# JeroendenBoef/GraphPOPE

Hardware: AMD Instinct MI355X
Metric: POPE embeddings/sec (nodes x anchors) + SAGE nodes/sec, Flickr 256 anchors (higher is better)
Workload: dtype u64; 1 GPU; configs[1]: flickr-shaped geodesic-stochastic, N=89250 E=899756 F=500, 256 anchors PER GPU (np.random seed 42); inputs resident in HBM (edge_index, x) -> [N, F+K] f32 in HBM on every rank; anchors_total=256, anchors_per_rank=256, parallelism=single GPU

## Files before the change

### graphpope_amd/_lib.py

```python
from __future__ import annotations

import ctypes
import os
from ctypes import c_char_p, c_double, c_float, c_int, c_int32, c_int64, c_size_t, c_uint64, c_void_p, POINTER

_HERE = os.path.dirname(os.path.abspath(__file__))
LIB_PATH = os.path.join(_HERE, "libgraphpope_hip.so")

OK, ERR_INVALID, ERR_HIP, ERR_INDEX, ERR_HOP_OVERFLOW, ERR_WORKSPACE, ERR_NO_DEVICE, ERR_UNSORTED = 0, -1, -2, -3, -4, -5, -6, -7
METRIC = {"distance": 0, "similarity": 1, "euclidean": 2}
KNOB_LIVE_MODE, KNOB_FINALIZE_VARIANT, KNOB_FINALIZE_BLOCKS = 0, 1, 2
KNOB_PAIRWISE_KERNEL, KNOB_COPY_BATCHES, KNOB_FAIL_HOST_REGISTER = 4, 5, 7
KNOB_SAGE_FORWARD_OVERLAP = 14
KNOB_GEMM_TILE16_BUFFERS = 18
KNOB_PREPARE_MERGE = 19
KNOB_STREAMK_XCD = 20
KNOB_FORWARD_WHOLE_TILES = 21

SIGNATURES = {
    "pope_last_error": (c_char_p, []),
    "pope_version": (c_char_p, []),
    "pope_require_device": (c_int, [POINTER(c_int32)]),
    "pope_debug_set": (c_int, [c_int32, c_int32]),
    "pope_host_copy_2d": (c_int, [c_void_p, c_int64, c_void_p, c_int64, c_int64, c_int64, c_int32]),
    "pope_copy_2d_to_host": (c_int, [c_void_p, c_int64, c_void_p, c_int64, c_int64, c_int64, c_void_p]),
    "pope_assemble_host_result": (c_int, [c_void_p, c_int64, c_int64, c_void_p, c_int64, c_int64, c_void_p, c_int64, c_int64, c_int32,
                                          c_int32, c_void_p]),
    "pope_assemble_begin": (c_void_p, [c_void_p, c_int64, c_int64, c_void_p, c_int64, c_int64, c_int32, c_int32]),
    "pope_assemble_finish": (c_int, [c_void_p, c_void_p, c_int64, c_int64, c_void_p]),
    "pope_assemble_abort": (None, [c_void_p]),
    "pope_assemble_prepare": (None, [c_int32]),
    "pope_assemble_ring_ready": (c_int32, []),
    "pope_assemble_finish_codes": (c_int, [c_void_p, c_void_p, c_int64, c_int32, c_void_p, c_void_p]),
    "pope_geodesic_hop_codes": (c_int, [c_void_p, c_int32, c_int32, c_int64, c_int32, c_void_p, c_int64, c_void_p, c_void_p]),
    "pope_host_pin": (c_int, [c_void_p, c_size_t]),
    "pope_host_unpin": (c_int, [c_void_p]),
    "pope_copy_to_device": (c_int, [c_void_p, c_void_p, c_size_t, c_void_p]),
    "pope_csr_scratch_bytes": (c_size_t, [c_int64, c_int64]),
    "pope_csr_aux_elems": (c_size_t, [c_int64]),
    "pope_csr_build": (c_int, [c_void_p, c_int64, c_int64, c_void_p, c_void_p, c_void_p, c_void_p, c_void_p, c_size_t,
# ... 15 lines not shown
    "pope_kmeans_lloyd_step": (c_int, [c_void_p, c_int64, c_int32, c_void_p, c_int32, c_void_p, c_void_p, c_void_p, c_void_p, c_void_p,
                                       c_void_p, c_size_t, c_void_p]),
    "pope_words": (c_int32, [c_int32]),
    "pope_plane_bytes": (c_size_t, [c_int64, c_int32]),
    "pope_bfs_scratch_bytes": (c_size_t, [c_int64, c_int64, c_int32]),
    "pope_geodesic_bfs": (c_int, [c_void_p, c_void_p, c_void_p, c_void_p, c_int64, c_int64, c_void_p, c_int32, c_void_p, c_int32,
                                  c_void_p, c_size_t, POINTER(c_int32), POINTER(c_int32), c_void_p]),
    "pope_geodesic_bfs_begin": (c_int, [c_void_p, c_void_p, c_void_p, c_void_p, c_int64, c_int64, c_void_p, c_int32, c_void_p, c_int32,
                                        c_void_p, c_size_t, c_void_p]),
    "pope_geodesic_bfs_finish": (c_int, [c_void_p, c_void_p, c_void_p, c_void_p, c_int64, c_int64, c_void_p, c_int32, c_void_p, c_int32,
                                         c_void_p, c_size_t, POINTER(c_int32), POINTER(c_int32), c_void_p]),
    "pope_geodesic_finalize": (c_int, [c_void_p, c_int32, c_int64, c_int32, c_void_p, c_int32, c_void_p, c_int64,
                                       c_int32, c_void_p]),
    "pope_geodesic_run_workspace_bytes": (c_size_t, [c_int64, c_int64, c_int32, c_int32]),
    "pope_geodesic_run_planes": (c_void_p, [c_void_p, c_int64, c_int64, c_int32, c_int32]),
    "pope_geodesic_run": (c_int, [c_void_p, c_int64, c_int64, c_void_p, c_int32, c_void_p, c_int32, c_void_p, c_int64,
                                  c_int32, c_void_p, c_size_t, POINTER(c_int32), POINTER(c_int32), c_void_p]),
    "pope_profile_levels": (None, [c_int32]),
    "pope_profile_read": (c_int32, [c_void_p, c_void_p, c_int32]),
    "pope_geodesic_finalize_shards": (c_int, [c_void_p, c_int32, c_int64, c_int32, c_int64, c_int32, c_void_p, c_int32,
                                              c_void_p, c_int64, c_void_p]),
    "pope_finalize_kernel_name": (c_int, [c_int64, c_int32, c_int32, c_int32, c_int32, c_char_p, c_size_t]),
    "pope_level_kernel_name": (c_int, [c_int64, c_int32, c_char_p, c_size_t]),
    "pope_column_stats_scratch_bytes": (c_size_t, [c_int32]),
    "pope_geodesic_column_stats": (c_int, [c_void_p, c_int32, c_int64, c_int32, c_void_p, c_void_p, c_void_p, c_size_t, c_void_p]),
    "pope_geodesic_hops": (c_int, [c_void_p, c_int32, c_int64, c_int32, c_void_p, c_void_p]),
    "pope_pairwise_scratch_bytes": (c_size_t, [c_int64, c_int32, c_int32]),
    "pope_pairwise_minmax": (c_int, [c_void_p, c_int64, c_int32, c_void_p, c_int32, c_int32, c_void_p, c_int64,
                                     c_int32, c_void_p, c_size_t, c_void_p]),
    "pope_pairwise_by_id_scratch_bytes": (c_size_t, [c_int64, c_int32, c_int32]),
    "pope_pairwise_features_by_id": (c_int, [c_void_p, c_int32, c_void_p, c_int64, c_int32, c_void_p, c_int32, c_int32, c_void_p, c_int64, c_int32,
                                             c_void_p, c_size_t, c_void_p]),
    "pope_pairwise_features": (c_int, [c_void_p, c_int32, c_void_p, c_int64, c_int32, c_void_p, c_int32, c_int32, c_void_p, c_int64,
                                       c_int32, c_void_p, c_size_t, c_void_p]),
    "pope_concat": (c_int, [c_void_p, c_int64, c_int32, c_void_p, c_int64, c_void_p]),
    "sage_conv_scratch_bytes": (c_size_t, [c_int64, c_int64, c_int64, c_int32, c_int32]),
    "sage_conv_forward_scratch_bytes": (c_size_t, [c_int64, c_int32, c_int32]),
    "sage_conv_forward": (c_int, [c_void_p, c_void_p, c_int64, c_int64, c_int64, c_void_p, c_int32, c_void_p,
                                  c_void_p, c_void_p, c_int32, c_void_p, c_void_p, c_void_p, c_size_t, c_void_p, c_void_p]),
    "sage_gather_mean": (c_int, [c_void_p, c_void_p, c_int64, c_int64, c_int64, c_void_p, c_int32, c_void_p, c_void_p]),
    "sage_conv_forward_indexed": (c_int, [c_void_p, c_void_p, c_void_p, c_int64, c_int64, c_int64, c_void_p, c_int64, c_int32,
                                          c_void_p, c_void_p, c_void_p, c_int32, c_void_p, c_void_p, c_void_p, c_void_p, c_size_t,
                                          c_void_p, c_void_p]),
    "sage_conv_forward_stats": (c_int, [c_void_p, c_void_p, c_int64, c_int64, c_int64, c_void_p, c_int32, c_void_p,
                                        c_void_p, c_void_p, c_int32, c_void_p, c_void_p, c_void_p, c_size_t, c_void_p, c_void_p, c_void_p, c_int32,
                                        c_void_p, c_void_p]),
# ... 110 lines not shown
```

### graphpope_amd/csrc/abi.cpp

```cpp
#include <cstring>

#include "common.h"

namespace pope {

static thread_local char g_error[512] = "";

void set_error(const char *fmt, ...) {
    va_list ap;
    va_start(ap, fmt);
    vsnprintf(g_error, sizeof(g_error), fmt, ap);
    va_end(ap);
}

void clear_error() { g_error[0] = '\0'; }

int g_fail_host_register = 0;

}

extern "C" const char *pope_last_error(void) { return pope::g_error; }

extern "C" const char *pope_version(void) { return "graphpope_hip 0.2 gfx950"; }

// ... 15 lines not shown
    }
    if (cu_count_host) *cu_count_host = prop.multiProcessorCount;
    return POPE_OK;
}

extern "C" int pope_debug_set(int32_t knob, int32_t value) {
    pope::clear_error();
    pope::FinalizeKnobs &fin = pope::g_geodesic.fin;
    switch (knob) {
    case POPE_KNOB_LIVE_MODE:        pope::g_geodesic.live_mode = value; break;
    case POPE_KNOB_FINALIZE_VARIANT:
        if (value >= 8 && value <= 10) { fin.variant = 1; fin.lut = value == 9 ? 2 : value == 8 ? 1 : 0; }
        else if (value == 11 || value == 12) fin.shard_batches = value == 11;
        else fin.variant = value;
        break;
    case POPE_KNOB_FINALIZE_BLOCKS:  fin.blocks = value > 0 ? value : 256 * 8; fin.blocks_set = value > 0; break;
    case POPE_KNOB_PAIRWISE_KERNEL:  pope::g_pairwise_kernel = value; break;
    case POPE_KNOB_COPY_BATCHES:     pope::g_copy_batches_per_wave = value; break;
    case POPE_KNOB_FAIL_HOST_REGISTER: pope::g_fail_host_register = value; break;
    case POPE_KNOB_SAGE_FORWARD_OVERLAP: pope::g_sage_forward_overlap = value != 0; break;
    case POPE_KNOB_GEMM_TILE16_BUFFERS: pope::g_gemm_tile16_buffers = value == 4 ? 4 : 3; break;
    case POPE_KNOB_FORWARD_WHOLE_TILES: pope::g_forward_whole_tiles = value != 0; break;
    case POPE_KNOB_PREPARE_MERGE:    pope::g_geodesic.prepare_merge = value; break;
    case POPE_KNOB_STREAMK_XCD:      pope::g_streamk_xcd = value != 0; break;
    default: pope::set_error("pope_debug_set: unknown knob %d", knob); return POPE_ERR_INVALID;
    }
    return POPE_OK;
}

extern "C" int pope_copy_2d_to_host(const void *src, int64_t src_pitch_bytes, void *dst_host, int64_t dst_pitch_bytes,
                                    int64_t row_bytes, int64_t rows, void *stream) {
    pope::clear_error();
    POPE_REQUIRE(src && dst_host, "pope_copy_2d_to_host: null pointer");
    POPE_REQUIRE(row_bytes > 0 && rows > 0 && src_pitch_bytes >= row_bytes && dst_pitch_bytes >= row_bytes, "pope_copy_2d_to_host: bad size");
    POPE_HIP(hipMemcpy2DAsync(dst_host, (size_t)dst_pitch_bytes, src, (size_t)src_pitch_bytes, (size_t)row_bytes, (size_t)rows,
                              hipMemcpyDeviceToHost, (hipStream_t)stream));
    return POPE_OK;
}
```

### graphpope_amd/csrc/common.h

```cpp
#pragma once

#include <hip/hip_runtime.h>

#include <atomic>
#include <cstdarg>
#include <cstdint>
#include <cstdio>

#include "graphpope_hip.h"

namespace pope {

typedef unsigned long long u64;

void set_error(const char *fmt, ...) __attribute__((format(printf, 1, 2)));
void clear_error();

inline int hip_fail(hipError_t e, const char *what, const char *file, int line) {
    set_error("%s failed: %s (%s:%d)", what, hipGetErrorString(e), file, line);
    return POPE_ERR_HIP;
}

#define POPE_HIP(call)                                                         \
    do {                                                                       \
        hipError_t e_ = (call);                                                \
        if (e_ != hipSuccess) return ::pope::hip_fail(e_, #call, __FILE__, __LINE__); \
    } while (0)

#define POPE_REQUIRE(cond, ...)                 \
    do {                                        \
        if (!(cond)) {                          \
            ::pope::set_error(__VA_ARGS__);     \
            return POPE_ERR_INVALID;            \
        }                                       \
    } while (0)

struct FinalizeKnobs {
    int variant = 1;
    int blocks = 256 * 8;
    bool blocks_set = false;
    int shard_batches = 1;
    int lut = 1;
};
struct GeodesicKnobs {
    int live_mode = -1;
    FinalizeKnobs fin;
    int prepare_merge = 1;
};
extern GeodesicKnobs g_geodesic;
extern int g_sage_forward_overlap, g_forward_whole_tiles, g_gemm_tile16_buffers, g_streamk_xcd;
extern int g_pairwise_kernel;
extern int g_copy_batches_per_wave;
extern int g_fail_host_register;

inline size_t align_up(size_t x, size_t a) { return (x + a - 1) / a * a; }

struct LdsOptIn {
    std::atomic<unsigned long long> mask[2] = {{0}, {0}};
    static int device() {
        int dev = 0;
        return hipGetDevice(&dev) == hipSuccess && dev >= 0 && dev < 128 ? dev : -1;
    }
    bool done() const {
        const int d = device();
        return d >= 0 && ((mask[d >> 6].load(std::memory_order_acquire) >> (d & 63)) & 1ull);
    }
    void mark() {
        const int d = device();
        if (d >= 0) mask[d >> 6].fetch_or(1ull << (d & 63), std::memory_order_release);
    }
// ... 32 lines not shown
```

### graphpope_amd/csrc/geodesic.hip

```cpp
#include <atomic>
#include <chrono>
#include <cstddef>
#include <cstring>
#include <mutex>
#include <type_traits>
#include <vector>

#include <rocprim/device/device_scan.hpp>
#include <rocprim/device/device_segmented_radix_sort.hpp>

#include "common.h"
#include "side_copy.h"

namespace pope {

enum { CSR_FLAG_BAD_INDEX = 1, CSR_FLAG_UNSORTED = 2 };
constexpr size_t CTL_BYTES = 4096;
enum { AUX_FLAGS = 2, AUX_HEADER = 16 };
constexpr int SLOTS = 4;
constexpr int CHUNK_SHIFT = 8, CHUNK = 1 << CHUNK_SHIFT;

__device__ __forceinline__ void seed_anchor(long long a, int j, int Wp, u64 *seen, u64 *front, unsigned *live) {
    const size_t idx = (size_t)a * Wp + (j >> 6);
    const u64 bit = 1ull << (j & 63);
    atomicOr(&seen[idx], bit);
    atomicOr(&front[idx], bit);
    atomicOr(&live[a >> 5], 1u << (a & 31));
}

__device__ __forceinline__ int csr_sorted_edge(int e, long long s, long long d, long long prev, const long long *__restrict__ src, int E, int N,
                                               int *__restrict__ rowptr, int *aux) {
    if (s < 0 || s >= N || d < 0 || d >= N) return CSR_FLAG_BAD_INDEX;
    int flags = 0;
    if (prev > s) {
        flags = CSR_FLAG_UNSORTED;
    } else if (prev >= -1 && prev < s) {
        for (long long r = prev + 1; r <= s; ++r) rowptr[r] = e;
    }
    if (e == E - 1)
        for (long long r = s + 1; r <= N; ++r) rowptr[r] = E;
    if ((e & (CHUNK - 1)) == 0) {
        const int c = e >> CHUNK_SHIFT;
        const bool first_continuation = c > 0 && prev == s && (c == 1 || src[e - CHUNK - 1] != s);
        aux[AUX_HEADER + c] = first_continuation ? (int)s : -1;
    }
    return flags;
}

template <bool PAIRS>
__device__ __forceinline__ int csr_sorted_role(const long long *__restrict__ src, const long long *__restrict__ dst, int E, int N,
                                               int *__restrict__ rowptr, int *__restrict__ col, int *__restrict__ erow, int *aux,
                                               const int bid, const int nblk) {
    int flags = 0;
    if (PAIRS) {
        typedef long long ll2 __attribute__((ext_vector_type(2)));
        for (int t = bid * blockDim.x + threadIdx.x; 2 * t < E; t += nblk * blockDim.x) {
            const int e = 2 * t;
            const ll2 s2 = reinterpret_cast<const ll2 *>(src)[t], d2 = reinterpret_cast<const ll2 *>(dst)[t];
            const long long prev = e > 0 ? src[e - 1] : -1;
            const int f0 = csr_sorted_edge(e, s2.x, d2.x, prev, src, E, N, rowptr, aux);
            const int f1 = csr_sorted_edge(e + 1, s2.y, d2.y, s2.x, src, E, N, rowptr, aux);
            flags |= f0 | f1;
            reinterpret_cast<int2 *>(col)[t] = make_int2((int)d2.x, (int)d2.y);
            reinterpret_cast<int2 *>(erow)[t] = make_int2((int)s2.x, (int)s2.y);
        }
    } else {
        for (int e = bid * blockDim.x + threadIdx.x; e < E; e += nblk * blockDim.x) {
            const long long s = src[e], d = dst[e];
            const int f = csr_sorted_edge(e, s, d, e > 0 ? src[e - 1] : -1, src, E, N, rowptr, aux);
            flags |= f;
            if (f & CSR_FLAG_BAD_INDEX) continue;
            col[e] = (int)d;
            erow[e] = (int)s;
        }
    }
    return flags;
}

template <bool PAIRS>
__global__ __launch_bounds__(256) void k_csr_sorted(const long long *__restrict__ src,
                                                    const long long *__restrict__ dst, int E, int N,
                                                    int *__restrict__ rowptr, int *__restrict__ col,
                                                    int *__restrict__ erow, int *aux,
                                                    const long long *__restrict__ anchors, int K, int Wp, u64 *seen,
                                                    u64 *front, unsigned *live) {
    const int seed_blocks = (K + (int)blockDim.x - 1) / (int)blockDim.x;
    if (K > 0 && (int)gridDim.x >= seed_blocks) {
        const int sb = (int)blockIdx.x - ((int)gridDim.x - seed_blocks);
        if (sb >= 0) {
            const int j = sb * (int)blockDim.x + (int)threadIdx.x;
            if (j < K) seed_anchor(anchors[j], j, Wp, seen, front, live);
        }
    } else if (K > 0 && blockIdx.x == gridDim.x - 1) {
        for (int j = threadIdx.x; j < K; j += blockDim.x) seed_anchor(anchors[j], j, Wp, seen, front, live);
    }
    const int flags = csr_sorted_role<PAIRS>(src, dst, E, N, rowptr, col, erow, aux, (int)blockIdx.x, (int)gridDim.x);
// ... 62 lines not shown
    const unsigned w = (unsigned)aux[AUX_FLAGS];
    return (w >> 3) == ctl->flag_epoch ? (int)(w & 7u) : 0;
}

__device__ __forceinline__ void csr_raise(int *aux, int flags, unsigned epoch) {
    if (epoch == 0) {
        atomicOr(&aux[AUX_FLAGS], flags);
        return;
    }
    unsigned *p = reinterpret_cast<unsigned *>(&aux[AUX_FLAGS]);
    unsigned old = *p;
    for (int tries = 0; tries < 1 << 20; ++tries) {
        const unsigned want = (old >> 3) == epoch ? old | (unsigned)flags : (epoch << 3) | (unsigned)flags;
        const unsigned seen = atomicCAS(p, old, want);
        if (seen == old) return;
        old = seen;
    }
}

__device__ __forceinline__ bool bfs_over(const BfsCtl *ctl, const int *aux, int level) {
    return ctl->last_active < level - 1 || csr_flags(ctl, aux) != 0;
}

constexpr int PREP_MAX_ANCHORS = 256;
struct PrepSeeds { int a[PREP_MAX_ANCHORS]; };

template <bool PAIRS>
__global__ __launch_bounds__(256) void k_prepare(const long long *__restrict__ src, const long long *__restrict__ dst, int E, int N,
                                                 int *__restrict__ rowptr, int *__restrict__ col, int *__restrict__ erow, int *aux,
                                                 uint4 *za, size_t na, uint4 *zb, size_t nb, u64 *zb_tail, int zero_blocks, unsigned epoch,
                                                 PrepSeeds seeds, int K, int Wp, u64 *seen, u64 *front, unsigned *live) {
    if ((int)blockIdx.x >= zero_blocks) {
        const int flags = csr_sorted_role<PAIRS>(src, dst, E, N, rowptr, col, erow, aux, (int)blockIdx.x - zero_blocks, (int)gridDim.x - zero_blocks);
        if (flags) csr_raise(aux, flags, epoch);
        return;
    }
    const uint4 z = make_uint4(0, 0, 0, 0);
    const size_t stride = (size_t)zero_blocks * blockDim.x, first = (size_t)blockIdx.x * blockDim.x + threadIdx.x;
    static_assert(offsetof(BfsCtl, flag_epoch) == 16, "k_prepare writes the tag as the first word of the control block's second unit");
    for (size_t i = first; i < na; i += stride) za[i] = i == 1 ? make_uint4(epoch, 0, 0, 0) : z;
    for (size_t i = first; i < nb; i += stride) zb[i] = z;
    if (zb_tail && first == 0) *zb_tail = 0;
    asm volatile("s_waitcnt vmcnt(0)" ::: "memory");
    __syncthreads();
    auto mine = [&](const void *word, const void *region) {
        const size_t u = (size_t)((const char *)word - (const char *)region) >> 4;
        return (u % stride) / blockDim.x == blockIdx.x;
    };
    for (int j = threadIdx.x; j < K; j += blockDim.x) {
        const long long a = seeds.a[j];
        const size_t idx = (size_t)a * Wp + (j >> 6);
        const u64 bit = 1ull << (j & 63);
        if (mine(&seen[idx], zb)) atomicOr(&seen[idx], bit);
        if (mine(&front[idx], za)) atomicOr(&front[idx], bit);
        if (mine(&live[a >> 5], za)) atomicOr(&live[a >> 5], 1u << (a & 31));
    }
}

__device__ __forceinline__ void raise_level(BfsCtl *ctl, int level) {
    if (__hip_atomic_load(&ctl->last_active, __ATOMIC_RELAXED, __HIP_MEMORY_SCOPE_AGENT) != level)
        __hip_atomic_store(&ctl->last_active, level, __ATOMIC_RELAXED, __HIP_MEMORY_SCOPE_AGENT);
}

__global__ __launch_bounds__(256) void k_zero(uint4 *a, size_t na, uint4 *b, size_t nb, uint4 *c, size_t nc, u64 *b_tail, uint4 *d, size_t nd,
                                              const long long *__restrict__ rows, int n_rows, u64 *row_base, int Wp) {
    const uint4 z = make_uint4(0, 0, 0, 0);
    const size_t stride = (size_t)gridDim.x * blockDim.x;
    if (b_tail && blockIdx.x == 0 && threadIdx.x == 0) *b_tail = 0;
    for (size_t i = (size_t)blockIdx.x * blockDim.x + threadIdx.x; i < nd; i += stride) d[i] = z;
    if (rows)
        for (size_t i = (size_t)blockIdx.x * blockDim.x + threadIdx.x; i < (size_t)n_rows * Wp; i += stride) row_base[(size_t)rows[i / Wp] * Wp + i % Wp] = 0;
    for (size_t i = (size_t)blockIdx.x * blockDim.x + threadIdx.x; i < na; i += stride) a[i] = z;
    for (size_t i = (size_t)blockIdx.x * blockDim.x + threadIdx.x; i < nb; i += stride) b[i] = z;
    for (size_t i = (size_t)blockIdx.x * blockDim.x + threadIdx.x; i < nc; i += stride) c[i] = z;
}

__global__ __launch_bounds__(256) void k_zero_words(u64 *p, size_t n) {
    for (size_t i = (size_t)blockIdx.x * blockDim.x + threadIdx.x; i < n; i += (size_t)gridDim.x * blockDim.x) p[i] = 0;
}

__global__ __launch_bounds__(256) void k_clear_spanning_rows(const int *__restrict__ aux, int nchunks, u64 *__restrict__ buf, int Wp) {
    const int *mrows = aux + AUX_HEADER;
    for (int i = blockIdx.x * blockDim.x + threadIdx.x; i < nchunks; i += gridDim.x * blockDim.x) {
        const int mv = mrows[i];
// ... 733 lines not shown
    case FIN_PIPE: snprintf(name, cap, "k_finalize_pipe<%d, %d>", p.xp, p.ep); break;
    case FIN_FAST: snprintf(name, cap, "k_finalize_fast"); break;
    default:       snprintf(name, cap, p.vec ? "k_finalize<true>" : "k_finalize<false>"); break;
    }
    return POPE_OK;
}

extern "C" int pope_geodesic_finalize(const uint64_t *planes, int32_t n_hop_bits, int64_t N, int32_t K,
                                      const float *x, int32_t F, float *out, int64_t out_cols, int32_t c0,
                                      void *stream_) {
    clear_error();
    POPE_REQUIRE(planes && out, "pope_geodesic_finalize: null pointer");
    POPE_REQUIRE(N > 0 && N < INT32_MAX && K > 0 && F >= 0 && c0 >= 0 && n_hop_bits >= 0 && n_hop_bits <= 31,
                 "pope_geodesic_finalize: bad size");
    POPE_REQUIRE(out_cols >= (int64_t)F + c0 + K, "pope_geodesic_finalize: out_cols %lld < F + c0 + K = %lld",
                 (long long)out_cols, (long long)F + c0 + K);
    return finalize_enqueue((const u64 *)planes, n_hop_bits, nullptr, N, K, x, F, out, out_cols, c0, (hipStream_t)stream_);
}

struct RunLayout {
    size_t rowptr, col, erow, aux, csr_scratch, planes, bfs_scratch, total;
};

static RunLayout run_layout(int64_t N, int64_t E, int32_t K, int32_t capacity) {
    RunLayout L;
    size_t o = 0;
    L.rowptr = o;      o += align_up((size_t)(N + 1) * sizeof(int), 256);
    L.col = o;         o += align_up((size_t)(E > 0 ? E : 1) * sizeof(int), 256);
    L.erow = o;        o += align_up((size_t)(E > 0 ? E : 1) * sizeof(int), 256);
    L.aux = o;         o += align_up(pope_csr_aux_elems(E) * sizeof(int), 256);
    L.csr_scratch = o; o += align_up(pope_csr_scratch_bytes(N, E), 256);
    L.planes = o;      o += align_up((size_t)(capacity + 1) * pope_plane_bytes(N, K), 256);
    L.bfs_scratch = o; o += align_up(pope_bfs_scratch_bytes(N, E, K), 256);
    L.total = o;
    return L;
}

extern "C" size_t pope_geodesic_run_workspace_bytes(int64_t N, int64_t E, int32_t K, int32_t plane_capacity) {
    if (N < 0 || E < 0 || K <= 0 || plane_capacity < 1 || plane_capacity > 31) return 0;
    return run_layout(N, E, K, plane_capacity).total;
}

extern "C" uint64_t *pope_geodesic_run_planes(void *workspace, int64_t N, int64_t E, int32_t K, int32_t plane_capacity) {
    if (!workspace || N < 0 || E < 0 || K <= 0 || plane_capacity < 1 || plane_capacity > 31) return nullptr;
    return (uint64_t *)((char *)workspace + run_layout(N, E, K, plane_capacity).planes);
}

extern "C" int pope_geodesic_run(const int64_t *edge_index, int64_t E, int64_t N, const int64_t *anchors_host, int32_t K,
                                 const float *x, int32_t F, float *out, int64_t out_cols, int32_t plane_capacity,
                                 void *workspace, size_t workspace_bytes, int32_t *max_hop_host,
                                 int32_t *n_hop_bits_host, void *stream_) {
    clear_error();
    hipStream_t stream = (hipStream_t)stream_;
    POPE_REQUIRE(N > 0 && N < INT32_MAX && E >= 0 && E < INT32_MAX && K > 0 && F >= 0, "pope_geodesic_run: bad size");
    POPE_REQUIRE(plane_capacity >= 1 && plane_capacity <= 31, "pope_geodesic_run: need 1 <= plane_capacity <= 31");
    POPE_REQUIRE(workspace && (edge_index || E == 0) && anchors_host, "pope_geodesic_run: null pointer");
    POPE_REQUIRE(!out || out_cols >= (int64_t)F + K, "pope_geodesic_run: out_cols %lld < F + K", (long long)out_cols);
    const RunLayout L = run_layout(N, E, K, plane_capacity);
    if (workspace_bytes < L.total) {
        set_error("pope_geodesic_run: workspace %zu < %zu bytes", workspace_bytes, L.total);
        return POPE_ERR_WORKSPACE;
    }
    char *ws = (char *)workspace;
    int *rowptr = (int *)(ws + L.rowptr), *col = (int *)(ws + L.col), *erow = (int *)(ws + L.erow), *aux = (int *)(ws + L.aux);
    u64 *planes = (u64 *)(ws + L.planes);
    int rc;
    Bfs b;
    b.slot = nullptr;
    SlotGuard guard{&b.slot, stream};
    if ((rc = bfs_setup(b, rowptr, col, erow, aux, N, E, anchors_host, K, (uint64_t *)planes, plane_capacity,
                        ws + L.bfs_scratch, L.total - L.bfs_scratch))) return rc;
    const int window = speculative_window(N, E, K);
    memcpy(b.slot->anchors, anchors_host, (size_t)K * sizeof(long long));
    if (g_geodesic.prepare_merge && K <= PREP_MAX_ANCHORS && E > 0) {
        static std::atomic<unsigned> epochs{0};
        unsigned epoch;
        do epoch = 0x10000000u | ((++epochs * 0x9E3779B1u) & 0x0fffffffu); while (epoch == 0x1fffffffu);
        PrepSeeds seeds;
        for (int j = 0; j < K; ++j) seeds.a[j] = (int)anchors_host[j];
        const int eager = b.capacity < EAGER_PLANES ? b.capacity : EAGER_PLANES;
        const size_t zwords = (size_t)(1 + eager) * b.plane_elems;
        const size_t na = (b.front_off + 3 * align_up(b.plane_bytes, 256) + 3 * live_bytes(b.N)) / 16, nb = zwords / 2;
        u64 *zb_tail = (zwords & 1) ? b.seen + zwords - 1 : nullptr;
        const long long *src = (const long long *)edge_index, *dst = src + E;
        const int zero_blocks = (g_geodesic.prepare_merge & 0xffff) > 1 ? (g_geodesic.prepare_merge & 0xffff) : 1024;
        const bool pairs = (E & 1) == 0 && ((reinterpret_cast<uintptr_t>(src) | reinterpret_cast<uintptr_t>(col) | reinterpret_cast<uintptr_t>(erow)) & 15u) == 0;
        unsigned csr_blocks = pairs ? capped_grid(E / 2, 256) : capped_grid(E, 256);
        if ((g_geodesic.prepare_merge >> 16) > 0) csr_blocks = std::min<unsigned>(csr_blocks, (unsigned)(g_geodesic.prepare_merge >> 16));
        if (pairs)
            hipLaunchKernelGGL(k_prepare<true>, dim3(zero_blocks + csr_blocks), dim3(256), 0, stream, src, dst, (int)E, (int)N, rowptr, col, erow, aux,
                               (uint4 *)b.base, na, (uint4 *)b.seen, nb, zb_tail, zero_blocks, epoch, seeds, K, b.Wp, b.seen, b.front[0], b.live[0]);
        else
            hipLaunchKernelGGL(k_prepare<false>, dim3(zero_blocks + csr_blocks), dim3(256), 0, stream, src, dst, (int)E, (int)N, rowptr, col, erow, aux,
                               (uint4 *)b.base, na, (uint4 *)b.seen, nb, zb_tail, zero_blocks, epoch, seeds, K, b.Wp, b.seen, b.front[0], b.live[0]);
        POPE_HIP(hipGetLastError());
        b.frontiers_cleared = true;
    } else {
        bfs_enqueue_clear(b, aux, stream);
        SeedArgs seed;
        seed.anchors = b.slot->anchors_dev; seed.K = K; seed.Wp = b.Wp; seed.seen = b.seen; seed.front = b.front[0]; seed.live = b.live[0];
        rc = csr_build(edge_index, E, N, rowptr, col, erow, aux, ws + L.csr_scratch, L.planes - L.csr_scratch, 2, seed, stream);
        if (rc) return rc;
    }
    int level = bfs_enqueue_levels(b, 1, 1 + window, stream);
    int ticket = 0;
    if (out) {
        ticket = b.slot->ticket = b.slot->ticket == INT32_MAX ? 1 : b.slot->ticket + 1;
        if ((rc = finalize_enqueue(planes, 0, &b.ctl->last_active, N, K, x, F, out, out_cols, 0, stream, 1, 0, aux,
                                   b.slot->report_dev, ticket))) return rc;
    }
    int last_active = 0;
    bool done = false;
    rc = bfs_poll(b, level, &last_active, &done, stream, ticket);
    if (rc == POPE_ERR_UNSORTED) {
        clear_error();
        if ((rc = csr_fallback((const long long *)edge_index, (const long long *)edge_index + E, (int)E, (int)N, rowptr, col,
                               erow, aux, ws + L.csr_scratch, stream))) return rc;
        b.frontiers_cleared = false;
        if ((rc = bfs_enqueue_init(b, anchors_host, stream))) return rc;
        level = 1;
        done = false;
    } else if (rc) {
        return rc;
    } else if (done) {
        guard.quiescent = true;
        remember_depth(N, E, K, last_active);
        if (max_hop_host) *max_hop_host = last_active;
        if (n_hop_bits_host) *n_hop_bits_host = hop_bits(last_active);
        return POPE_OK;
    }
    while (!done) {
        level = bfs_enqueue_levels(b, level, level + LEVEL_BATCH, stream);
        if ((rc = bfs_poll(b, level, &last_active, &done, stream))) return rc;
    }
    if (out && (rc = finalize_enqueue(planes, hop_bits(last_active), nullptr, N, K, x, F, out, out_cols, 0, stream))) return rc;
    guard.quiescent = true;
    remember_depth(N, E, K, last_active, window < LEVEL_BATCH);
    if (max_hop_host) *max_hop_host = last_active;
    if (n_hop_bits_host) *n_hop_bits_host = hop_bits(last_active);
    return POPE_OK;
}

extern "C" int pope_geodesic_finalize_shards(const uint64_t *planes, int32_t n_shards, int64_t shard_stride_words,
                                             int32_t n_hop_bits, int64_t N, int32_t K_shard, const float *x, int32_t F,
                                             float *out, int64_t out_cols, void *stream_) {
    clear_error();
// ... 76 lines not shown
```

### include/graphpope_hip.h

```cpp
#ifndef GRAPHPOPE_HIP_H
#define GRAPHPOPE_HIP_H

#include <stddef.h>
#include <stdint.h>

#ifdef __cplusplus
extern "C" {
#endif

#define POPE_OK                 0
#define POPE_ERR_INVALID       -1
#define POPE_ERR_HIP           -2
#define POPE_ERR_INDEX         -3
#define POPE_ERR_HOP_OVERFLOW  -4
#define POPE_ERR_WORKSPACE     -5
#define POPE_ERR_NO_DEVICE     -6
#define POPE_ERR_UNSORTED      -7

const char *pope_last_error(void);

const char *pope_version(void);

int pope_require_device(int32_t *cu_count_host);

#define POPE_KNOB_LIVE_MODE         0
#define POPE_KNOB_FINALIZE_VARIANT  1
#define POPE_KNOB_FINALIZE_BLOCKS   2
#define POPE_KNOB_PAIRWISE_KERNEL   4
#define POPE_KNOB_COPY_BATCHES      5
#define POPE_KNOB_FAIL_HOST_REGISTER 7
#define POPE_KNOB_SAGE_FORWARD_OVERLAP 14
#define POPE_KNOB_GEMM_TILE16_BUFFERS 18
#define POPE_KNOB_PREPARE_MERGE     19
#define POPE_KNOB_STREAMK_XCD       20
#define POPE_KNOB_FORWARD_WHOLE_TILES 21
int pope_debug_set(int32_t knob, int32_t value);

size_t pope_csr_scratch_bytes(int64_t N, int64_t E);
size_t pope_csr_aux_elems(int64_t E);

int pope_csr_build(const int64_t *edge_index, int64_t E, int64_t N, int32_t *rowptr, int32_t *col, int32_t *erow,
                   int32_t *aux, void *scratch, size_t scratch_bytes, int32_t defer_check, void *stream);

int pope_csr_build_canonical(const int64_t *edge_index, int64_t E, int64_t N, int32_t *rowptr, int32_t *col, int32_t *erow,
                             int32_t *aux, void *scratch, size_t scratch_bytes, void *stream);

int pope_pagerank_weights(const int32_t *rowptr, const int32_t *col, int64_t N, double *w, void *stream);
int pope_pagerank_step(const int32_t *rowptr_by_target, const int32_t *sources, int64_t N, const double *x, const double *w,
                       double dangling_sum, double alpha, double *x_out, void *stream);

size_t pope_clustering_scratch_bytes(int64_t N, int64_t E);
int pope_clustering_counts(const int32_t *rowptr, const int32_t *col, const int32_t *erow, const int32_t *rowptr_by_target,
                           const int32_t *sources, const int32_t *erow_by_target, int64_t N, int64_t E, int64_t *T, int64_t *dt,
                           int64_t *db, void *scratch, size_t scratch_bytes, void *stream);

size_t pope_betweenness_scratch_bytes(int64_t N, int64_t batch);
int pope_betweenness_batch(const int32_t *rowptr, const int32_t *col, int64_t E_by_source, const int32_t *rowptr_by_target,
                           const int32_t *sources, int64_t E_by_target, int64_t N, int64_t first_source, int64_t num_sources,
// ... 19 lines not shown
int pope_geodesic_bfs(const int32_t *rowptr, const int32_t *col, const int32_t *erow, const int32_t *aux,
                      int64_t N, int64_t E,
                      const int64_t *anchors_host, int32_t K, uint64_t *planes, int32_t plane_capacity, void *scratch, size_t scratch_bytes,
                      int32_t *max_hop_host, int32_t *n_hop_bits_host, void *stream);

int pope_geodesic_bfs_begin(const int32_t *rowptr, const int32_t *col, const int32_t *erow, const int32_t *aux,
                            int64_t N, int64_t E, const int64_t *anchors_host, int32_t K, uint64_t *planes,
                            int32_t plane_capacity, void *scratch, size_t scratch_bytes, void *stream);
int pope_geodesic_bfs_finish(const int32_t *rowptr, const int32_t *col, const int32_t *erow, const int32_t *aux,
                             int64_t N, int64_t E, const int64_t *anchors_host, int32_t K, uint64_t *planes,
                             int32_t plane_capacity, void *scratch, size_t scratch_bytes, int32_t *max_hop_host,
                             int32_t *n_hop_bits_host, void *stream);

int pope_geodesic_finalize(const uint64_t *planes, int32_t n_hop_bits, int64_t N, int32_t K_shard,
                           const float *x, int32_t F, float *out, int64_t out_cols, int32_t c0, void *stream);

int pope_geodesic_finalize_shards(const uint64_t *planes, int32_t n_shards, int64_t shard_stride_words, int32_t n_hop_bits,
                                  int64_t N, int32_t K_shard, const float *x, int32_t F, float *out, int64_t out_cols,
                                  void *stream);

int pope_finalize_kernel_name(int64_t N, int32_t K_shard, int32_t F, int32_t has_x, int32_t n_shards, char *name, size_t cap);

int pope_level_kernel_name(int64_t N, int32_t K, char *name, size_t cap);

size_t pope_geodesic_run_workspace_bytes(int64_t N, int64_t E, int32_t K, int32_t plane_capacity);
uint64_t *pope_geodesic_run_planes(void *workspace, int64_t N, int64_t E, int32_t K, int32_t plane_capacity);
int pope_geodesic_run(const int64_t *edge_index, int64_t E, int64_t N, const int64_t *anchors_host, int32_t K,
                      const float *x, int32_t F, float *out, int64_t out_cols, int32_t plane_capacity,
                      void *workspace, size_t workspace_bytes, int32_t *max_hop_host, int32_t *n_hop_bits_host,
                      void *stream);

void pope_profile_levels(int32_t enable);
int32_t pope_profile_read(int32_t *levels_host, float *level_ms_host, int32_t capacity);

int pope_geodesic_hops(const uint64_t *planes, int32_t n_hop_bits, int64_t N, int32_t K,
                       int32_t *hops, void *stream);

size_t pope_column_stats_scratch_bytes(int32_t K);
int pope_geodesic_column_stats(const uint64_t *planes, int32_t n_hop_bits, int64_t N, int32_t K, int64_t *hop_sum,
                               int64_t *reach, void *scratch, size_t scratch_bytes, void *stream);

#define POPE_METRIC_COSINE_DISTANCE   0
#define POPE_METRIC_COSINE_SIMILARITY 1
#define POPE_METRIC_EUCLIDEAN         2

size_t pope_pairwise_scratch_bytes(int64_t N, int32_t K, int32_t D);
// ... 159 lines not shown
```

Baseline: 101.1 billion embeddings/s.

## Fold BFS level 1 into the merged CSR-build prepare kernel

While building the CSR, each block records edges whose destination is an anchor into a per-block list. The last-arriving block, found through a sharded arrival counter, then expands level 1 of the BFS frontier from those lists, so the BFS level loop can start at level 2. This removes one level kernel launch and its pass over the graph. In exchange it adds atomics, a grid-wide last-block election, extra scratch, and a fallback that re-runs from level 1 when a list overflows.

```diff
diff --git a/graphpope_amd/_lib.py b/graphpope_amd/_lib.py
--- a/graphpope_amd/_lib.py
+++ b/graphpope_amd/_lib.py
@@ -16,6 +16,7 @@
 KNOB_PREPARE_MERGE = 19
 KNOB_STREAMK_XCD = 20
 KNOB_FORWARD_WHOLE_TILES = 21
+KNOB_FOLD_LEVEL1, KNOB_LEVEL1_LIST_CAP = 22, 23
 
 SIGNATURES = {
     "pope_last_error": (c_char_p, []),
@@ -77,6 +78,7 @@
                                               c_void_p, c_int64, c_void_p]),
     "pope_finalize_kernel_name": (c_int, [c_int64, c_int32, c_int32, c_int32, c_int32, c_char_p, c_size_t]),
     "pope_level_kernel_name": (c_int, [c_int64, c_int32, c_char_p, c_size_t]),
+    "pope_geodesic_run_plan_name": (c_int, [c_int64, c_int64, c_int32, c_int32, c_int32, c_int32, c_char_p, c_size_t]),
     "pope_column_stats_scratch_bytes": (c_size_t, [c_int32]),
     "pope_geodesic_column_stats": (c_int, [c_void_p, c_int32, c_int64, c_int32, c_void_p, c_void_p, c_void_p, c_size_t, c_void_p]),
     "pope_geodesic_hops": (c_int, [c_void_p, c_int32, c_int64, c_int32, c_void_p, c_void_p]),
diff --git a/graphpope_amd/csrc/abi.cpp b/graphpope_amd/csrc/abi.cpp
--- a/graphpope_amd/csrc/abi.cpp
+++ b/graphpope_amd/csrc/abi.cpp
@@ -61,6 +61,8 @@
     case POPE_KNOB_GEMM_TILE16_BUFFERS: pope::g_gemm_tile16_buffers = value == 4 ? 4 : 3; break;
     case POPE_KNOB_FORWARD_WHOLE_TILES: pope::g_forward_whole_tiles = value != 0; break;
     case POPE_KNOB_PREPARE_MERGE:    pope::g_geodesic.prepare_merge = value; break;
+    case POPE_KNOB_FOLD_LEVEL1:      pope::g_geodesic.fold_level1 = value != 0; break;
+    case POPE_KNOB_LEVEL1_LIST_CAP:  pope::g_geodesic.level1_list_cap = value > 0 ? value : 0; break;
     case POPE_KNOB_STREAMK_XCD:      pope::g_streamk_xcd = value != 0; break;
     default: pope::set_error("pope_debug_set: unknown knob %d", knob); return POPE_ERR_INVALID;
     }
diff --git a/graphpope_amd/csrc/common.h b/graphpope_amd/csrc/common.h
--- a/graphpope_amd/csrc/common.h
+++ b/graphpope_amd/csrc/common.h
@@ -46,6 +46,8 @@
     int live_mode = -1;
     FinalizeKnobs fin;
     int prepare_merge = 1;
+    int fold_level1 = 1;
+    int level1_list_cap = 0;
 };
 extern GeodesicKnobs g_geodesic;
 extern int g_sage_forward_overlap, g_forward_whole_tiles, g_gemm_tile16_buffers, g_streamk_xcd;
diff --git a/graphpope_amd/csrc/geodesic.hip b/graphpope_amd/csrc/geodesic.hip
--- a/graphpope_amd/csrc/geodesic.hip
+++ b/graphpope_amd/csrc/geodesic.hip
@@ -1,3 +1,4 @@
+#include <algorithm>
 #include <atomic>
 #include <chrono>
 #include <cstddef>
@@ -14,7 +15,8 @@
 
 namespace pope {
 
-enum { CSR_FLAG_BAD_INDEX = 1, CSR_FLAG_UNSORTED = 2 };
+enum { CSR_FLAG_BAD_INDEX = 1, CSR_FLAG_UNSORTED = 2,
+       CSR_FLAG_L1_OVERFLOW = 4 };
 constexpr size_t CTL_BYTES = 4096;
 enum { AUX_FLAGS = 2, AUX_HEADER = 16 };
 constexpr int SLOTS = 4;
@@ -47,10 +49,11 @@
     return flags;
 }
 
-template <bool PAIRS>
+struct NoEdgeHook { __device__ __forceinline__ void operator()(long long, long long) const {} };
+template <bool PAIRS, class OnEdge = NoEdgeHook>
 __device__ __forceinline__ int csr_sorted_role(const long long *__restrict__ src, const long long *__restrict__ dst, int E, int N,
                                                int *__restrict__ rowptr, int *__restrict__ col, int *__restrict__ erow, int *aux,
-                                               const int bid, const int nblk) {
+                                               const int bid, const int nblk, OnEdge on_edge = OnEdge()) {
     int flags = 0;
     if (PAIRS) {
         typedef long long ll2 __attribute__((ext_vector_type(2)));
@@ -63,6 +66,8 @@
             flags |= f0 | f1;
             reinterpret_cast<int2 *>(col)[t] = make_int2((int)d2.x, (int)d2.y);
             reinterpret_cast<int2 *>(erow)[t] = make_int2((int)s2.x, (int)s2.y);
+            on_edge(s2.x, d2.x);
+            on_edge(s2.y, d2.y);
         }
     } else {
         for (int e = bid * blockDim.x + threadIdx.x; e < E; e += nblk * blockDim.x) {
@@ -72,6 +77,7 @@
             if (f & CSR_FLAG_BAD_INDEX) continue;
             col[e] = (int)d;
             erow[e] = (int)s;
+            on_edge(s, d);
         }
     }
     return flags;
@@ -180,23 +186,205 @@
     return ctl->last_active < level - 1 || csr_flags(ctl, aux) != 0;
 }
 
+__device__ __forceinline__ void raise_level(BfsCtl *ctl, int level) {
+    if (__hip_atomic_load(&ctl->last_active, __ATOMIC_RELAXED, __HIP_MEMORY_SCOPE_AGENT) != level)
+        __hip_atomic_store(&ctl->last_active, level, __ATOMIC_RELAXED, __HIP_MEMORY_SCOPE_AGENT);
+}
+
 constexpr int PREP_MAX_ANCHORS = 256;
 struct PrepSeeds { int a[PREP_MAX_ANCHORS]; };
+
+constexpr int L1_SHARDS = 64;
+constexpr int L1_LINE_WORDS = 16;
+constexpr int L1_MAX_BLOCKS = 4096;
+constexpr int L1_MAX_SEGMENT = 2048;
+constexpr int L1_MAX_TOTAL = 16384;
+constexpr unsigned L1_COUNT_OVERFLOW = 0x80000000u;
+struct L1Fold {
+    int on;
+    int seg_cap, total_cap;
+    int Wp, N;
+    u64 *arrive;
+    unsigned *counts;
+    u64 *pairs;
+    u64 *front1;
+    unsigned *live1;
+    size_t wt_lo[3], wt_hi[3];
+    int sorted[PREP_MAX_ANCHORS];
+};
+struct L1Shared {
+    int sorted[PREP_MAX_ANCHORS];
+    u64 bits[PREP_MAX_ANCHORS * 4];
+    unsigned short pre[L1_MAX_BLOCKS];
+    int wave_sum[4];
+    int hits, last, total, over;
+};
+
+__device__ __forceinline__ int l1_lower_bound(const int *sorted, int x) {
+    int lo = 0;
+#pragma unroll
+    for (int step = PREP_MAX_ANCHORS / 2; step; step >>= 1)
+        if (sorted[lo + step - 1] < x) lo += step;
+    return lo;
+}
+
+__device__ __forceinline__ bool l1_arrive(u64 *word, unsigned epoch, unsigned expected, bool *stuck) {
+    u64 old = __hip_atomic_load(word, __ATOMIC_RELAXED, __HIP_MEMORY_SCOPE_AGENT);
+    for (int tries = 0; tries < 1 << 20; ++tries) {
+        const u64 want = (unsigned)(old >> 32) == epoch ? old + 1 : ((u64)epoch << 32) | 1u;
+        const u64 seen = atomicCAS(word, old, want);
+        if (seen == old) return (unsigned)want == expected;
+        old = seen;
+    }
+    *stuck = true;
+    return false;
+}
+
+__device__ __forceinline__ bool l1_block_arrives(const L1Fold &f, unsigned epoch, int *aux) {
+    const unsigned G = gridDim.x, shard = blockIdx.x % L1_SHARDS;
+    const unsigned in_shard = G / L1_SHARDS + (shard < G % L1_SHARDS ? 1u : 0u), shards = G < (unsigned)L1_SHARDS ? G : (unsigned)L1_SHARDS;
+    bool stuck = false;
+    bool last = l1_arrive(f.arrive + (size_t)shard * L1_LINE_WORDS, epoch, in_shard, &stuck);
+    if (last) last = l1_arrive(f.arrive + (size_t)L1_SHARDS * L1_LINE_WORDS, epoch, shards, &stuck);
+    if (stuck) csr_raise(aux, CSR_FLAG_L1_OVERFLOW, epoch);
+    return last;
+}
+
+__device__ __forceinline__ void l1_last_block(const L1Fold &f, const PrepSeeds &seeds, int K, int csr_blocks, unsigned epoch, BfsCtl *ctl, int *aux,
+                                              L1Shared &sh) {
+    const int tid = threadIdx.x, lane = tid & 63, wv = tid >> 6;
+    __builtin_amdgcn_fence(__ATOMIC_ACQUIRE, "agent");
+    unsigned c[L1_MAX_BLOCKS / 256];
+#pragma unroll
+    for (int k = 0; k < L1_MAX_BLOCKS / 256; ++k) {
+        const int b = k * 256 + tid;
+        c[k] = __hip_atomic_load(f.counts + (b < csr_blocks ? b : 0), __ATOMIC_RELAXED, __HIP_MEMORY_SCOPE_AGENT);
+        if (b >= csr_blocks) c[k] = 0u;
+    }
+    sh.sorted[tid] = f.sorted[tid];
+#pragma unroll
+    for (int i = 0; i < 4; ++i) sh.bits[tid * 4 + i] = 0;
+    if (tid == 0) sh.over = 0;
+    __syncthreads();
+    bool over = false;
+#pragma unroll
+    for (int k = 0; k < L1_MAX_BLOCKS / 256; ++k) {
+        over |= c[k] > (unsigned)f.seg_cap;
+        sh.pre[k * 256 + tid] = (unsigned short)(over ? 0u : c[k]);
+    }
+    if (over) sh.over = 1;
+    if (tid < K) atomicOr(&sh.bits[l1_lower_bound(sh.sorted, seeds.a[tid]) * 4 + (tid >> 6)], 1ull << (tid & 63));
+    __syncthreads();
+    constexpr int PER = L1_MAX_BLOCKS / 256;
+    int own = 0;
+    for (int k = 0; k < PER; ++k) own += sh.pre[tid * PER + k];
+    int incl = own;
+#pragma unroll
+    for (int d = 1; d < 64; d <<= 1) {
+        const int up = __shfl_up(incl, d);
+        if (lane >= d) incl += up;
+    }
+    if (lane == 63) sh.wave_sum[wv] = incl;
+    __syncthreads();
+    int base = incl - own;
+    for (int w = 0; w < wv; ++w) base += sh.wave_sum[w];
+    const int total = sh.wave_sum[0] + sh.wave_sum[1] + sh.wave_sum[2] + sh.wave_sum[3];
+    if (sh.over || total > f.total_cap) {
+        if (tid == 0) csr_raise(aux, CSR_FLAG_L1_OVERFLOW, epoch);
+        return;
+    }
+    for (int k = 0; k < PER; ++k) {
+        const int n = sh.pre[tid * PER + k];
+        sh.pre[tid * PER + k] = (unsigned short)base;
+        base += n;
+    }
+    __syncthreads();
+    bool found = false;
+    constexpr int BATCH = 4;
+    for (int i0 = tid; i0 < total; i0 += 256 * BATCH) {
+        u64 pr[BATCH];
+#pragma unroll
+        for (int j = 0; j < BATCH; ++j) {
+            const int i = min(i0 + 256 * j, total - 1);
+            int p = 0;
+#pragma unroll
+            for (int step = L1_MAX_BLOCKS / 2; step; step >>= 1)
+                if ((int)sh.pre[p + step] <= i) p += step;
+            pr[j] = __hip_atomic_load(f.pairs + (size_t)p * f.seg_cap + (i - (int)sh.pre[p]), __ATOMIC_RELAXED, __HIP_MEMORY_SCOPE_AGENT);
+        }
+#pragma unroll
+        for (int j = 0; j < BATCH; ++j) {
+            if (i0 + 256 * j >= total) continue;
+            const int v = (int)(pr[j] >> 32), u = (int)(unsigned)pr[j];
+            const int iu = l1_lower_bound(sh.sorted, u), iv = l1_lower_bound(sh.sorted, v);
+            if (sh.sorted[iu] != u || v < 0 || v >= f.N) continue;
+            const bool v_anchor = sh.sorted[iv] == v;
+            u64 any = 0;
+            for (int w = 0; w < f.Wp; ++w) {
+                const u64 fresh = sh.bits[iu * 4 + w] & ~(v_anchor ? sh.bits[iv * 4 + w] : 0ull);
+                if (fresh) atomicOr(&f.front1[(size_t)v * f.Wp + w], fresh);
+                any |= fresh;
+            }
+            if (any) {
+                atomicOr(&f.live1[v >> 5], 1u << (v & 31));
+                found = true;
+            }
+        }
+    }
+    if (__any(found) && lane == 0) raise_level(ctl, 1);
+}
 
 template <bool PAIRS>
 __global__ __launch_bounds__(256) void k_prepare(const long long *__restrict__ src, const long long *__restrict__ dst, int E, int N,
                                                  int *__restrict__ rowptr, int *__restrict__ col, int *__restrict__ erow, int *aux,
                                                  uint4 *za, size_t na, uint4 *zb, size_t nb, u64 *zb_tail, int zero_blocks, unsigned epoch,
-                                                 PrepSeeds seeds, int K, int Wp, u64 *seen, u64 *front, unsigned *live) {
+                                                 PrepSeeds seeds, int K, int Wp, u64 *seen, u64 *front, unsigned *live, L1Fold fold) {
+    __shared__ L1Shared sh;
     if ((int)blockIdx.x >= zero_blocks) {
-        const int flags = csr_sorted_role<PAIRS>(src, dst, E, N, rowptr, col, erow, aux, (int)blockIdx.x - zero_blocks, (int)gridDim.x - zero_blocks);
+        const int bid = (int)blockIdx.x - zero_blocks, nblk = (int)gridDim.x - zero_blocks;
+        int flags;
+        if (fold.on) {
+            sh.sorted[threadIdx.x] = fold.sorted[threadIdx.x];
+            if (threadIdx.x == 0) sh.hits = 0;
+            __syncthreads();
+            u64 *segment = fold.pairs + (size_t)bid * fold.seg_cap;
+            flags = csr_sorted_role<PAIRS>(src, dst, E, N, rowptr, col, erow, aux, bid, nblk, [&](long long s, long long d) {
+                if ((unsigned long long)s >= (unsigned long long)N || (unsigned long long)d >= (unsigned long long)N) return;
+                if (sh.sorted[l1_lower_bound(sh.sorted, (int)d)] != (int)d) return;
+                const int pos = atomicAdd(&sh.hits, 1);
+                if (pos < fold.seg_cap)
+                    __hip_atomic_store(segment + pos, ((u64)(unsigned)s << 32) | (unsigned)d, __ATOMIC_RELAXED, __HIP_MEMORY_SCOPE_AGENT);
+            });
+        } else {
+            flags = csr_sorted_role<PAIRS>(src, dst, E, N, rowptr, col, erow, aux, bid, nblk);
+        }
         if (flags) csr_raise(aux, flags, epoch);
+        if (!fold.on) return;
+        asm volatile("s_waitcnt vmcnt(0)" ::: "memory");
+        __syncthreads();
+        if (threadIdx.x == 0) {
+            const unsigned n = (unsigned)sh.hits;
+            __hip_atomic_store(fold.counts + bid, n > (unsigned)fold.seg_cap ? L1_COUNT_OVERFLOW : n, __ATOMIC_RELAXED, __HIP_MEMORY_SCOPE_AGENT);
+            asm volatile("s_waitcnt vmcnt(0)" ::: "memory");
+            sh.last = l1_block_arrives(fold, epoch, aux) ? 1 : 0;
+        }
+        __syncthreads();
+        if (sh.last) l1_last_block(fold, seeds, K, nblk, epoch, reinterpret_cast<BfsCtl *>(za), aux, sh);
         return;
     }
     const uint4 z = make_uint4(0, 0, 0, 0);
     const size_t stride = (size_t)zero_blocks * blockDim.x, first = (size_t)blockIdx.x * blockDim.x + threadIdx.x;
     static_assert(offsetof(BfsCtl, flag_epoch) == 16, "k_prepare writes the tag as the first word of the control block's second unit");
-    for (size_t i = first; i < na; i += stride) za[i] = i == 1 ? make_uint4(epoch, 0, 0, 0) : z;
+    for (size_t i = first; i < na; i += stride) {
+        const uint4 val = i == 1 ? make_uint4(epoch, 0, 0, 0) : z;
+        if ((i >= fold.wt_lo[0] && i < fold.wt_hi[0]) || (i >= fold.wt_lo[1] && i < fold.wt_hi[1]) || (i >= fold.wt_lo[2] && i < fold.wt_hi[2])) {
+            u64 *p = reinterpret_cast<u64 *>(za + i);
+            __hip_atomic_store(p, (u64)val.x, __ATOMIC_RELAXED, __HIP_MEMORY_SCOPE_AGENT);
+            __hip_atomic_store(p + 1, (u64)0, __ATOMIC_RELAXED, __HIP_MEMORY_SCOPE_AGENT);
+        } else {
+            za[i] = val;
+        }
+    }
     for (size_t i = first; i < nb; i += stride) zb[i] = z;
     if (zb_tail && first == 0) *zb_tail = 0;
     asm volatile("s_waitcnt vmcnt(0)" ::: "memory");
@@ -213,11 +401,10 @@
         if (mine(&front[idx], za)) atomicOr(&front[idx], bit);
         if (mine(&live[a >> 5], za)) atomicOr(&live[a >> 5], 1u << (a & 31));
     }
-}
-
-__device__ __forceinline__ void raise_level(BfsCtl *ctl, int level) {
-    if (__hip_atomic_load(&ctl->last_active, __ATOMIC_RELAXED, __HIP_MEMORY_SCOPE_AGENT) != level)
-        __hip_atomic_store(&ctl->last_active, level, __ATOMIC_RELAXED, __HIP_MEMORY_SCOPE_AGENT);
+    if (!fold.on) return;
+    if (threadIdx.x == 0) sh.last = l1_block_arrives(fold, epoch, aux) ? 1 : 0;
+    __syncthreads();
+    if (sh.last) l1_last_block(fold, seeds, K, (int)gridDim.x - zero_blocks, epoch, reinterpret_cast<BfsCtl *>(za), aux, sh);
 }
 
 __global__ __launch_bounds__(256) void k_zero(uint4 *a, size_t na, uint4 *b, size_t nb, uint4 *c, size_t nc, u64 *b_tail, uint4 *d, size_t nd,
@@ -997,6 +1184,14 @@
     size_t rowptr, col, erow, aux, csr_scratch, planes, bfs_scratch, total;
 };
 
+constexpr int L1_MIN_SEGMENT = 256;
+static size_t l1_counts_off() { return align_up((size_t)(L1_SHARDS + 1) * L1_LINE_WORDS * sizeof(u64), 256); }
+static size_t l1_pairs_off(int64_t E) { return l1_counts_off() + align_up((size_t)capped_grid((size_t)E, 256) * sizeof(unsigned), 256); }
+static size_t run_csr_scratch_bytes(int64_t N, int64_t E) {
+    const size_t l1 = l1_pairs_off(E) + (size_t)capped_grid((size_t)E, 256) * L1_MIN_SEGMENT * sizeof(u64);
+    return align_up(std::max(pope_csr_scratch_bytes(N, E), l1), 256);
+}
+
 static RunLayout run_layout(int64_t N, int64_t E, int32_t K, int32_t capacity) {
     RunLayout L;
     size_t o = 0;
@@ -1004,7 +1199,7 @@
     L.col = o;         o += align_up((size_t)(E > 0 ? E : 1) * sizeof(int), 256);
     L.erow = o;        o += align_up((size_t)(E > 0 ? E : 1) * sizeof(int), 256);
     L.aux = o;         o += align_up(pope_csr_aux_elems(E) * sizeof(int), 256);
-    L.csr_scratch = o; o += align_up(pope_csr_scratch_bytes(N, E), 256);
+    L.csr_scratch = o; o += run_csr_scratch_bytes(N, E);
     L.planes = o;      o += align_up((size_t)(capacity + 1) * pope_plane_bytes(N, K), 256);
     L.bfs_scratch = o; o += align_up(pope_bfs_scratch_bytes(N, E, K), 256);
     L.total = o;
@@ -1019,6 +1214,52 @@
 extern "C" uint64_t *pope_geodesic_run_planes(void *workspace, int64_t N, int64_t E, int32_t K, int32_t plane_capacity) {
     if (!workspace || N < 0 || E < 0 || K <= 0 || plane_capacity < 1 || plane_capacity > 31) return nullptr;
     return (uint64_t *)((char *)workspace + run_layout(N, E, K, plane_capacity).planes);
+}
+
+struct RunKnobs { int prepare_merge, fold_level1, level1_list_cap; };
+struct RunPlan {
+    bool merged, fold_l1;
+    int first_level, stop_level;
+    bool finalize_in_stream;
+    size_t list_entries;
+    int total_cap;
+    size_t counts_off, pairs_off;
+};
+static RunPlan run_plan(int64_t N, int64_t E, int K, bool has_out, int window, const RunKnobs &knobs, size_t csr_scratch_bytes, int level_limit) {
+    RunPlan p{};
+    p.merged = knobs.prepare_merge != 0 && K <= PREP_MAX_ANCHORS && E > 0;
+    p.finalize_in_stream = has_out;
+    p.first_level = 1;
+    p.stop_level = E == 0 ? 1 : std::min(1 + window, level_limit);
+    if (p.merged && knobs.fold_level1 != 0) {
+        const size_t max_blocks = capped_grid((size_t)E, 256);
+        p.counts_off = l1_counts_off();
+        p.pairs_off = l1_pairs_off(E);
+        p.total_cap = knobs.level1_list_cap > 0 ? std::min(knobs.level1_list_cap, L1_MAX_TOTAL) : L1_MAX_TOTAL;
+        p.list_entries = csr_scratch_bytes > p.pairs_off ? (csr_scratch_bytes - p.pairs_off) / sizeof(u64) : 0;
+        p.fold_l1 = p.list_entries >= max_blocks && max_blocks <= (size_t)L1_MAX_BLOCKS;
+        if (p.fold_l1) p.first_level = 2;
+    }
+    if (p.stop_level < p.first_level) p.stop_level = p.first_level;
+    return p;
+}
+
+static RunKnobs run_knobs() { return RunKnobs{g_geodesic.prepare_merge, g_geodesic.fold_level1, g_geodesic.level1_list_cap}; }
+
+extern "C" int pope_geodesic_run_plan_name(int64_t N, int64_t E, int32_t K, int32_t F, int32_t has_out, int32_t hinted_depth, char *name, size_t cap) {
+    clear_error();
+    POPE_REQUIRE(name && cap > 0 && N > 0 && N < INT32_MAX && E >= 0 && E < INT32_MAX && K > 0 && F >= 0, "pope_geodesic_run_plan_name: bad argument");
+    const int window = hinted_depth > 0 ? std::min(LEVEL_BATCH, hinted_depth + 1) : LEVEL_BATCH;
+    const RunPlan p = run_plan(N, E, K, has_out != 0, window, run_knobs(), run_csr_scratch_bytes(N, E), 1 << 30);
+    char fin[64] = "k_bfs_report", levels[48] = "-";
+    if (has_out) {
+        int rc = pope_finalize_kernel_name(N, K, F, F > 0, 1, fin, sizeof(fin));
+        if (rc) return rc;
+    }
+    if (p.stop_level - p.first_level == 1) snprintf(levels, sizeof(levels), "L%d", p.first_level);
+    else if (p.stop_level > p.first_level) snprintf(levels, sizeof(levels), "L%d..L%d", p.first_level, p.stop_level - 1);
+    snprintf(name, cap, "%s | %s | %s", !p.merged ? "k_zero, k_csr_sorted" : p.fold_l1 ? "k_prepare+L1" : "k_prepare", levels, fin);
+    return POPE_OK;
 }
 
 extern "C" int pope_geodesic_run(const int64_t *edge_index, int64_t E, int64_t N, const int64_t *anchors_host, int32_t K,
@@ -1046,8 +1287,9 @@
     if ((rc = bfs_setup(b, rowptr, col, erow, aux, N, E, anchors_host, K, (uint64_t *)planes, plane_capacity,
                         ws + L.bfs_scratch, L.total - L.bfs_scratch))) return rc;
     const int window = speculative_window(N, E, K);
+    const RunPlan plan = run_plan(N, E, K, out != nullptr, window, run_knobs(), L.planes - L.csr_scratch, (int)std::min<long long>(b.level_limit, 1 << 30));
     memcpy(b.slot->anchors, anchors_host, (size_t)K * sizeof(long long));
-    if (g_geodesic.prepare_merge && K <= PREP_MAX_ANCHORS && E > 0) {
+    if (plan.merged) {
         static std::atomic<unsigned> epochs{0};
         unsigned epoch;
         do epoch = 0x10000000u | ((++epochs * 0x9E3779B1u) & 0x0fffffffu); while (epoch == 0x1fffffffu);
@@ -1062,12 +1304,33 @@
         const bool pairs = (E & 1) == 0 && ((reinterpret_cast<uintptr_t>(src) | reinterpret_cast<uintptr_t>(col) | reinterpret_cast<uintptr_t>(erow)) & 15u) == 0;
         unsigned csr_blocks = pairs ? capped_grid(E / 2, 256) : capped_grid(E, 256);
         if ((g_geodesic.prepare_merge >> 16) > 0) csr_blocks = std::min<unsigned>(csr_blocks, (unsigned)(g_geodesic.prepare_merge >> 16));
+        L1Fold fold{};
+        if (plan.fold_l1) {
+            char *region = ws + L.csr_scratch;
+            fold.on = 1;
+            fold.seg_cap = (int)std::min<size_t>(plan.list_entries / csr_blocks, (size_t)std::min(L1_MAX_SEGMENT, plan.total_cap));
+            fold.total_cap = plan.total_cap;
+            fold.Wp = b.Wp; fold.N = b.N;
+            fold.arrive = (u64 *)region;
+            fold.counts = (unsigned *)(region + plan.counts_off);
+            fold.pairs = (u64 *)(region + plan.pairs_off);
+            fold.front1 = b.front[1]; fold.live1 = b.live[1];
+            const auto unit = [&](const void *q) { return (size_t)((const char *)q - b.base) / 16; };
+            fold.wt_lo[0] = 0;                fold.wt_hi[0] = CTL_BYTES / 16;
+            fold.wt_lo[1] = unit(b.front[1]); fold.wt_hi[1] = unit(b.front[2]);
+            fold.wt_lo[2] = unit(b.live[1]);  fold.wt_hi[2] = unit(b.live[2]);
+            int n = 0;
+            for (int j = 0; j < K; ++j) fold.sorted[n++] = seeds.a[j];
+            std::sort(fold.sorted, fold.sorted + n);
+            n = (int)(std::unique(fold.sorted, fold.sorted + n) - fold.sorted);
+            for (; n < PREP_MAX_ANCHORS; ++n) fold.sorted[n] = INT32_MAX;
+        }
         if (pairs)
             hipLaunchKernelGGL(k_prepare<true>, dim3(zero_blocks + csr_blocks), dim3(256), 0, stream, src, dst, (int)E, (int)N, rowptr, col, erow, aux,
-                               (uint4 *)b.base, na, (uint4 *)b.seen, nb, zb_tail, zero_blocks, epoch, seeds, K, b.Wp, b.seen, b.front[0], b.live[0]);
+                               (uint4 *)b.base, na, (uint4 *)b.seen, nb, zb_tail, zero_blocks, epoch, seeds, K, b.Wp, b.seen, b.front[0], b.live[0], fold);
         else
             hipLaunchKernelGGL(k_prepare<false>, dim3(zero_blocks + csr_blocks), dim3(256), 0, stream, src, dst, (int)E, (int)N, rowptr, col, erow, aux,
-                               (uint4 *)b.base, na, (uint4 *)b.seen, nb, zb_tail, zero_blocks, epoch, seeds, K, b.Wp, b.seen, b.front[0], b.live[0]);
+                               (uint4 *)b.base, na, (uint4 *)b.seen, nb, zb_tail, zero_blocks, epoch, seeds, K, b.Wp, b.seen, b.front[0], b.live[0], fold);
         POPE_HIP(hipGetLastError());
         b.frontiers_cleared = true;
     } else {
@@ -1077,7 +1340,7 @@
         rc = csr_build(edge_index, E, N, rowptr, col, erow, aux, ws + L.csr_scratch, L.planes - L.csr_scratch, 2, seed, stream);
         if (rc) return rc;
     }
-    int level = bfs_enqueue_levels(b, 1, 1 + window, stream);
+    int level = bfs_enqueue_levels(b, plan.first_level, plan.stop_level, stream);
     int ticket = 0;
     if (out) {
         ticket = b.slot->ticket = b.slot->ticket == INT32_MAX ? 1 : b.slot->ticket + 1;
@@ -1097,6 +1360,11 @@
         done = false;
     } else if (rc) {
         return rc;
+    } else if (b.slot->report[1] & CSR_FLAG_L1_OVERFLOW) {
+        b.frontiers_cleared = false;
+        if ((rc = bfs_enqueue_init(b, anchors_host, stream))) return rc;
+        level = 1;
+        done = false;
     } else if (done) {
         guard.quiescent = true;
         remember_depth(N, E, K, last_active);
diff --git a/include/graphpope_hip.h b/include/graphpope_hip.h
--- a/include/graphpope_hip.h
+++ b/include/graphpope_hip.h
@@ -34,6 +34,8 @@
 #define POPE_KNOB_PREPARE_MERGE     19
 #define POPE_KNOB_STREAMK_XCD       20
 #define POPE_KNOB_FORWARD_WHOLE_TILES 21
+#define POPE_KNOB_FOLD_LEVEL1      22
+#define POPE_KNOB_LEVEL1_LIST_CAP  23
 int pope_debug_set(int32_t knob, int32_t value);
 
 size_t pope_csr_scratch_bytes(int64_t N, int64_t E);
@@ -99,6 +101,8 @@
 int pope_finalize_kernel_name(int64_t N, int32_t K_shard, int32_t F, int32_t has_x, int32_t n_shards, char *name, size_t cap);
 
 int pope_level_kernel_name(int64_t N, int32_t K, char *name, size_t cap);
+
+int pope_geodesic_run_plan_name(int64_t N, int64_t E, int32_t K, int32_t F, int32_t has_out, int32_t hinted_depth, char *name, size_t cap);
 
 size_t pope_geodesic_run_workspace_bytes(int64_t N, int64_t E, int32_t K, int32_t plane_capacity);
 uint64_t *pope_geodesic_run_planes(void *workspace, int64_t N, int64_t E, int32_t K, int32_t plane_capacity);
```

After: 85.63 billion embeddings/s. -15.3%, worse.
